# jrnerupudinho/Semi-Blind-Channel-Estimation-for-MIMO-RIS-communication-system-Using-EM-Algo

Hardware: NVIDIA B200
Metric: EM channel-estimation trials/sec (higher is better)
Workload: dtype f64

## Files before the change

semi-blind-channel-estimation-for-mimo-ris-communication-system-using-em-algo_b200/csrc/estep.cu:

```cuda
#include <math.h>

#include "common.cuh"
#include "tensor.cuh"

namespace sbce {

static __device__ __forceinline__ constexpr int cmax(int a, int b) { return a > b ? a : b; }

__global__ void k_pilot_stats(int n_tx, int total, const cplx* __restrict__ Xp, cplx* __restrict__ pm,
                              cplx* __restrict__ pR) {
    int s = blockIdx.x * blockDim.x + threadIdx.x;
    if (s >= total) return;
    const cplx* x = Xp + (size_t)s * n_tx;
    for (int i = 0; i < n_tx; ++i) {
        cplx xi = x[i];
        pm[(size_t)s * n_tx + i] = cconj(xi);
        for (int j = 0; j < n_tx; ++j) pR[((size_t)s * n_tx + i) * n_tx + j] = cmulc(x[j], xi);
    }
}

cudaError_t launch_pilot_stats(const Dims& d, int nb, const double* Xp, double* pil_m, double* pil_R, cudaStream_t s) {
    int total = nb * d.T_p;
    if (total == 0) return cudaSuccess;
    k_pilot_stats<<<(total + 127) / 128, 128, 0, s>>>(d.n_tx, total, (const cplx*)Xp, (cplx*)pil_m, (cplx*)pil_R);
    count_launch();
    return cudaGetLastError();
}

template <int NTX, int NRX>
__device__ __forceinline__ void heff_qr_finish(const Dims& d, int b, int t, cplx (&A)[cmax(NTX, NRX)][NTX],
                                               const cplx* __restrict__ Yd, const cplx* __restrict__ Xoff,
                                               double* __restrict__ qr) {
    constexpr int NR = cmax(NTX, NRX);
    cplx y[NR];
#pragma unroll
    for (int r = 0; r < NR; ++r) y[r] = (r < NRX) ? Yd[((size_t)b * d.T_d + t) * NRX + r] : mk(0.0, 0.0);
    if (Xoff != nullptr) {
        const cplx* o = Xoff + ((size_t)b * d.T_d + t) * NTX;
#pragma unroll
        for (int j = 0; j < NTX; ++j) {
            const cplx oj = o[j], noj = mk(-oj.x, -oj.y);
#pragma unroll
            for (int r = 0; r < NRX; ++r) cfma(y[r], A[r][j], noj);
        }
    }

#pragma unroll
    for (int k = 0; k < NTX; ++k) {
        double nrm2 = 0.0;
#pragma unroll
        for (int i = k; i < NR; ++i) nrm2 += cnorm2(A[i][k]);
        if (nrm2 > 0.0) {
            const double nrm = sqrt(nrm2);
            const cplx a0 = A[k][k];
            const double abs0 = sqrt(cnorm2(a0));
            const cplx phase = abs0 > 0.0 ? mk(a0.x / abs0, a0.y / abs0) : mk(1.0, 0.0);
            const cplx vk = cscale(phase, abs0 + nrm);
            const double beta = 1.0 / (nrm * (nrm + abs0));
#pragma unroll
            for (int c = k + 1; c <= NTX; ++c) {
                cplx w = mk(0.0, 0.0);
                if (c < NTX) {
                    cfmac(w, A[k][c], vk);
#pragma unroll
                    for (int i = k + 1; i < NR; ++i) cfmac(w, A[i][c], A[i][k]);
                    w = cscale(w, beta);
                    cplx nw = mk(-w.x, -w.y);
                    cfma(A[k][c], nw, vk);
#pragma unroll
                    for (int i = k + 1; i < NR; ++i) cfma(A[i][c], nw, A[i][k]);
                } else {
                    cfmac(w, y[k], vk);
#pragma unroll
                    for (int i = k + 1; i < NR; ++i) cfmac(w, y[i], A[i][k]);
                    w = cscale(w, beta);
                    cplx nw = mk(-w.x, -w.y);
                    cfma(y[k], nw, vk);
#pragma unroll
                    for (int i = k + 1; i < NR; ++i) cfma(y[i], nw, A[i][k]);
                }
            }
            const cplx rot = mk(-phase.x, phase.y);
#pragma unroll
            for (int c = k + 1; c < NTX; ++c) A[k][c] = cmul(A[k][c], rot);
            y[k] = cmul(y[k], rot);
            A[k][k] = mk(nrm, 0.0);
        } else {
            A[k][k] = mk(0.0, 0.0);
        }
    }

    double* rec = qr + ((size_t)b * d.T_d + t) * d.rec;
    int o = 0;
#pragma unroll
    for (int i = 0; i < NTX; ++i)
#pragma unroll
        for (int j = i; j < NTX; ++j) {
            rec[o++] = A[i][j].x;
            rec[o++] = (j == i) ? 0.0 : A[i][j].y;
        }
#pragma unroll
    for (int i = 0; i < NTX; ++i) {
        rec[o++] = y[i].x;
        rec[o++] = y[i].y;
    }
    double c0 = 0.0;
#pragma unroll
    for (int i = NTX; i < NR; ++i) c0 += cnorm2(y[i]);
    rec[o++] = c0;
    rec[o++] = 0.0;
}

template <int NTX, int NRX>
__global__ void __launch_bounds__(128) k_heff_qr(Dims d, const cplx* __restrict__ Yd, const cplx* __restrict__ PsiD,
                                                 const cplx* __restrict__ theta, const int32_t* __restrict__ active,
                                                 const cplx* __restrict__ Xoff, double* __restrict__ qr, int use_smem) {
    constexpr int NR = cmax(NTX, NRX);
    extern __shared__ double2 heff_smem[];
    const int b = blockIdx.y;
    if (active != nullptr && active[b] == 0) return;
    const cplx* th = theta + (size_t)b * d.L * NRX;
    if (use_smem) {
        for (int e = threadIdx.x; e < d.L * NRX; e += blockDim.x) heff_smem[e] = th[e];
        __syncthreads();
        th = heff_smem;
    }
    const int t = blockIdx.x * blockDim.x + threadIdx.x;
    if (t >= d.T_d) return;

    const cplx* psi = PsiD + ((size_t)(d.psi_shared ? 0 : b) * d.T_d + t) * d.N1;

    cplx A[NR][NTX];
#pragma unroll
    for (int r = 0; r < NR; ++r)
#pragma unroll
        for (int j = 0; j < NTX; ++j) A[r][j] = mk(0.0, 0.0);

#pragma unroll 4
    for (int n = 0; n < d.N1; ++n) {
        const cplx p = psi[n];
        const cplx* row = th + (size_t)n * NTX * NRX;
#pragma unroll
        for (int j = 0; j < NTX; ++j)
#pragma unroll
            for (int r = 0; r < NRX; ++r) cfma(A[r][j], p, row[j * NRX + r]);
    }
    heff_qr_finish<NTX, NRX>(d, b, t, A, Yd, Xoff, qr);
}

template <int NTX, int NRX>
__global__ void __launch_bounds__(128, 4) k_heff_qr_mma(Dims d, const cplx* __restrict__ Yd,
                                                        const cplx* __restrict__ PsiD, const cplx* __restrict__ theta,
                                                        const int32_t* __restrict__ active,
                                                        const cplx* __restrict__ Xoff, double* __restrict__ qr) {
    constexpr int NR = cmax(NTX, NRX);
    constexpr int NC = NTX * NRX;
    constexpr int NT = (NC + 7) / 8;
    constexpr int TS = NT * 8 + 2;
    constexpr int HS = NC + 1;
    extern __shared__ double2 heff_smem[];
    const int b = blockIdx.y;
    if (active != nullptr && active[b] == 0) return;
    const int N1 = d.N1, KP = (N1 + 7) & ~7;
    cplx* sTh = heff_smem;
    cplx* sH = sTh + KP * TS;
    {
        const cplx* th = theta + (size_t)b * d.L * NRX;
        for (int e = threadIdx.x; e < KP * TS; e += blockDim.x) {
            const int n = e / TS, c = e % TS;
            sTh[e] = (n < N1 && c < NC) ? th[n * NC + c] : mk(0.0, 0.0);
        }
    }
    __syncthreads();
    const int warp = threadIdx.x >> 5, lane = threadIdx.x & 31, g = lane >> 2, tig = lane & 3;
    const int t0 = blockIdx.x * 128 + warp * 32;
    if (t0 >= d.T_d) return;
    const cplx* psi_b = PsiD + (size_t)(d.psi_shared ? 0 : b) * d.T_d * N1;
    const cplx* prow[2][2];
#pragma unroll
    for (int mt = 0; mt < 2; ++mt)
#pragma unroll
        for (int h = 0; h < 2; ++h) prow[mt][h] = psi_b + (size_t)min(t0 + mt * 16 + g + 8 * h, d.T_d - 1) * N1;
    {
        const char* rowp = (const char*)(psi_b + (size_t)min(t0 + lane, d.T_d - 1) * N1);
        for (int o = 0; o < N1 * (int)sizeof(cplx); o += 128) asm volatile("prefetch.global.L2 [%0];" ::"l"(rowp + o));
    }
    double cr[2][NT][4], ci[2][NT][4];
#pragma unroll
    for (int mt = 0; mt < 2; ++mt)
#pragma unroll
        for (int nt = 0; nt < NT; ++nt)
#pragma unroll
            for (int e = 0; e < 4; ++e) { cr[mt][nt][e] = 0.0; ci[mt][nt][e] = 0.0; }
#pragma unroll 2
    for (int k0 = 0; k0 < KP; k0 += 8) {
        const int ka = k0 + tig, kb = ka + 4;
        const bool va = ka < N1, vb = kb < N1;
        double ar[2][4], ai[2][4];
#pragma unroll
        for (int mt = 0; mt < 2; ++mt) {
            const cplx a0 = va ? prow[mt][0][ka] : mk(0.0, 0.0), a1 = va ? prow[mt][1][ka] : mk(0.0, 0.0);
            const cplx a2 = vb ? prow[mt][0][kb] : mk(0.0, 0.0), a3 = vb ? prow[mt][1][kb] : mk(0.0, 0.0);
            ar[mt][0] = a0.x; ar[mt][1] = a1.x; ar[mt][2] = a2.x; ar[mt][3] = a3.x;
            ai[mt][0] = a0.y; ai[mt][1] = a1.y; ai[mt][2] = a2.y; ai[mt][3] = a3.y;
        }
#pragma unroll
        for (int nt = 0; nt < NT; ++nt) {
            const cplx b0 = sTh[ka * TS + 8 * nt + g], b1 = sTh[kb * TS + 8 * nt + g];
#pragma unroll
            for (int mt = 0; mt < 2; ++mt) {
                dmma16x8x8(cr[mt][nt], ar[mt], b0.x, b1.x);
                dmma16x8x8(ci[mt][nt], ar[mt], b0.y, b1.y);
                dmma16x8x8(cr[mt][nt], ai[mt], -b0.y, -b1.y);
                dmma16x8x8(ci[mt][nt], ai[mt], b0.x, b1.x);
            }
        }
    }
    cplx* H = sH + (size_t)warp * 32 * HS;
#pragma unroll
    for (int mt = 0; mt < 2; ++mt)
#pragma unroll
        for (int nt = 0; nt < NT; ++nt)
#pragma unroll
            for (int h = 0; h < 2; ++h) {
                const int row = mt * 16 + g + 8 * h, c = 8 * nt + 2 * tig;
                if (c < NC) H[row * HS + c] = mk(cr[mt][nt][2 * h], ci[mt][nt][2 * h]);
                if (c + 1 < NC) H[row * HS + c + 1] = mk(cr[mt][nt][2 * h + 1], ci[mt][nt][2 * h + 1]);
            }
    __syncwarp();
    const int t = t0 + lane;
    if (t >= d.T_d) return;
    cplx A[NR][NTX];
#pragma unroll
    for (int r = 0; r < NR; ++r)
#pragma unroll
        for (int j = 0; j < NTX; ++j) A[r][j] = (r < NRX) ? H[lane * HS + j * NRX + r] : mk(0.0, 0.0);
    heff_qr_finish<NTX, NRX>(d, b, t, A, Yd, Xoff, qr);
}

__device__ __forceinline__ double group8_sum(double v) {
    v += shfl_xor_d(v, 4);
    v += shfl_xor_d(v, 2);
    v += shfl_xor_d(v, 1);
    return v;
}

template <int NTX>
__global__ void __launch_bounds__(128) k_heff_qr_rows(Dims d, const cplx* __restrict__ Yd,
                                                      const cplx* __restrict__ PsiD, const cplx* __restrict__ theta,
                                                      const int32_t* __restrict__ active,
                                                      const cplx* __restrict__ Xoff, double* __restrict__ qr) {
    const int b = blockIdx.y;
    if (active != nullptr && active[b] == 0) return;
    const int r = threadIdx.x & 7;
    const int tq = blockIdx.x * (blockDim.x >> 3) + (threadIdx.x >> 3);
    const bool tv = tq < d.T_d;
    const int t = tv ? tq : d.T_d - 1;
    const int nrx = d.n_rx;
    const bool rv = r < nrx;
    const int rr = rv ? r : 0;

    const cplx* psi = PsiD + ((size_t)(d.psi_shared ? 0 : b) * d.T_d + t) * d.N1;
    const cplx* th = theta + (size_t)b * d.L * nrx;

    cplx A[NTX + 1];
#pragma unroll
    for (int j = 0; j <= NTX; ++j) A[j] = mk(0.0, 0.0);
#pragma unroll 2
    for (int n = 0; n < d.N1; ++n) {
        const cplx p = psi[n];
        const cplx* row = th + (size_t)n * NTX * nrx + rr;
#pragma unroll
        for (int j = 0; j < NTX; ++j) cfma(A[j], p, __ldg(&row[j * nrx]));
    }
    A[NTX] = Yd[((size_t)b * d.T_d + t) * nrx + rr];
    if (Xoff != nullptr) {
        const cplx* o = Xoff + ((size_t)b * d.T_d + t) * NTX;
#pragma unroll
        for (int j = 0; j < NTX; ++j) {
            const cplx oj = o[j];
            cfma(A[NTX], A[j], mk(-oj.x, -oj.y));
        }
    }
    if (!rv) {
#pragma unroll
        for (int j = 0; j <= NTX; ++j) A[j] = mk(0.0, 0.0);
    }

#pragma unroll
    for (int k = 0; k < NTX; ++k) {
        const double nrm2 = group8_sum(r >= k ? cnorm2(A[k]) : 0.0);
        const bool ok = nrm2 > 0.0;
        const double nrm = sqrt(nrm2);
        const int src = (threadIdx.x & 24) + k;
        const cplx a0 = mk(shfl_d(A[k].x, src), shfl_d(A[k].y, src));
        const double abs0 = sqrt(cnorm2(a0));
        const cplx phase = abs0 > 0.0 ? mk(a0.x / abs0, a0.y / abs0) : mk(1.0, 0.0);
        const cplx vk = cscale(phase, abs0 + nrm);
        const double beta = ok ? 1.0 / (nrm * (nrm + abs0)) : 0.0;
        const cplx vr = (r == k) ? vk : (r > k ? A[k] : mk(0.0, 0.0));
#pragma unroll
        for (int c = k + 1; c <= NTX; ++c) {
            cplx w = mk(0.0, 0.0);
            cfmac(w, A[c], vr);
            w = mk(group8_sum(w.x) * beta, group8_sum(w.y) * beta);
            const cplx nw = mk(-w.x, -w.y);
            cfma(A[c], nw, vr);
        }
        if (r == k) {
            const cplx rot = mk(-phase.x, phase.y);
#pragma unroll
            for (int c = k + 1; c <= NTX; ++c) A[c] = cmul(A[c], rot);
            A[k] = mk(ok ? nrm : 0.0, 0.0);
        }
    }
    const double c0 = group8_sum(r >= NTX ? cnorm2(A[NTX]) : 0.0);
    if (!tv) return;
    double* rec = qr + ((size_t)b * d.T_d + t) * d.rec;
    if (r < NTX) {
        double* o = rec + 2 * (r * NTX - (r * (r - 1)) / 2);
#pragma unroll
        for (int j = 0; j < NTX; ++j)
            if (j >= r) {
                o[2 * (j - r)] = A[j].x;
                o[2 * (j - r) + 1] = (j == r) ? 0.0 : A[j].y;
            }
        rec[NTX * (NTX + 1) + 2 * r] = A[NTX].x;
        rec[NTX * (NTX + 1) + 2 * r + 1] = A[NTX].y;
    }
    if (r == 0) {
        rec[NTX * (NTX + 1) + 2 * NTX] = c0;
        rec[NTX * (NTX + 1) + 2 * NTX + 1] = 0.0;
    }
}

constexpr double SBCE_THR = 64.0;
constexpr int ENUM_QCAP = 1024;

template <int NTX, int SQM>
struct EnumT {
    static constexpr int M = SQM * SQM;
    static constexpr int BITS = (SQM == 2 ? 2 : (SQM == 4 ? 4 : 6));
    static constexpr int HB = BITS / 2;
    static constexpr int NODE_STREAMS = NTX - 1;
    static constexpr int PLWANT = (5 + BITS - 1) / BITS;
    static constexpr int PL = NODE_STREAMS < PLWANT ? NODE_STREAMS : PLWANT;
    static constexpr int NPREF = 1 << (BITS * PL);
    static constexpr int NPAIR = NTX * (NTX - 1) / 2;
    static constexpr int NPAIR1 = NPAIR > 0 ? NPAIR : 1;
    static constexpr int NACC = 1 + 3 * NTX + 2 * NPAIR;
    static constexpr int O_TAB = 0;
    static constexpr int O_G = O_TAB + 2 * NPAIR1 * M;
    static constexpr int O_YT = O_G + NTX * SQM;
    static constexpr int O_C0 = O_YT + 2 * NTX;
    static constexpr int O_ACC = O_C0 + 1;
    static constexpr int O_AREF = O_ACC + NACC;
    static constexpr int O_S2 = O_AREF + 1;
    static constexpr int O_CNT = O_S2 + 1;
    static constexpr int O_Q = O_CNT + 1;
    static constexpr int O_SCR = O_Q + ENUM_QCAP / 2;
    static constexpr int WS_DOUBLES = ((O_SCR + NACC * 32) + 1) & ~1;

    __device__ __forceinline__ static double pam(int a) { return (double)(2 * a - SQM + 1); }
    __device__ __forceinline__ static cplx cval(int m) { return mk(pam(m & (SQM - 1)), pam(m >> HB)); }
    __device__ __forceinline__ static int pair(int i, int s) { return s * (s - 1) / 2 + i; }

    __device__ __forceinline__ static int slice(double v, const double* gs, double& dist) {
        int a = 0;
        double e = v - gs[0];
        dist = e * e;
#pragma unroll
        for (int q = 1; q < SQM; ++q) {
            e = v - gs[q];
            const double dq = e * e;
            if (dq < dist) { dist = dq; a = q; }
        }
        return a;
    }

    __device__ __forceinline__ static double fold(double v, double r) {
        double a = fabs(v);
        if (SQM == 8) a = fabs(a - 4.0 * r);
        if (SQM >= 4) a = fabs(a - 2.0 * r);
        return a - r;
    }
};

template <int NTX, int SQM>
__device__ __noinline__ void enum_flush(double* ws, double warp_best) {
    typedef EnumT<NTX, SQM> E;
    constexpr int M = E::M;
    const int lane = threadIdx.x & 31;
    __syncwarp();
    int* cntp = (int*)(ws + E::O_CNT);
    const int n = min(*cntp, ENUM_QCAP);
    const int* q = (const int*)(ws + E::O_Q);
    const cplx* tab = (const cplx*)(ws + E::O_TAB);
    const double* g = ws + E::O_G;
    const double inv_s2 = ws[E::O_S2];
    double aref = ws[E::O_AREF];
    if (warp_best < aref) {
        const double f = exp((warp_best - aref) * inv_s2);
        for (int i = lane; i < E::NACC; i += 32) ws[E::O_ACC + i] *= f;
        aref = warp_best;
    }
    double* A = ws + E::O_ACC;
    if (n <= 2) {
        constexpr int LG = (SQM == 2 ? 1 : (SQM == 4 ? 2 : 3));
        const int a = lane & (SQM - 1);
        const bool isQ = (lane >> LG) & 1;
        const double pq = E::pam(a);
        for (int e = 0; e < n; ++e) {
            const int code = q[e];
            double base = ws[E::O_C0];
            cplx t0;
            {
                cplx acc[NTX];
#pragma unroll
                for (int i = 0; i < NTX; ++i) acc[i] = mk(ws[E::O_YT + 2 * i], ws[E::O_YT + 2 * i + 1]);
#pragma unroll
                for (int s = NTX - 1; s >= 1; --s) {
                    const int m = (code >> (E::BITS * (NTX - 1 - s))) & (M - 1);
                    const double eI = acc[s].x - g[s * SQM + (m & (SQM - 1))];
                    const double eQ = acc[s].y - g[s * SQM + (m >> E::HB)];
                    base += fma(eI, eI, eQ * eQ);
#pragma unroll
                    for (int i = 0; i < NTX; ++i)
                        if (i < s) acc[i] = csub(acc[i], tab[E::pair(i, s) * M + m]);
                }
                t0 = acc[0];
            }
            const double ev = (isQ ? t0.y : t0.x) - g[a];
            const double dd = ev * ev;
            double mn = dd;
#pragma unroll
            for (int o = SQM / 2; o > 0; o >>= 1) mn = fmin(mn, shfl_xor_d(mn, o));
            const double w = exp((mn - dd) * inv_s2);
            double s0 = w, s1 = pq * w, s2 = pq * pq * w;
#pragma unroll
            for (int o = SQM / 2; o > 0; o >>= 1) {
                s0 += shfl_xor_d(s0, o);
                s1 += shfl_xor_d(s1, o);
                s2 += shfl_xor_d(s2, o);
            }
            const double o0 = shfl_xor_d(s0, SQM), o1 = shfl_xor_d(s1, SQM), o2 = shfl_xor_d(s2, SQM);
            const double om = shfl_xor_d(mn, SQM);
            const double EI = isQ ? o0 : s0, A1 = isQ ? o1 : s1, A2 = isQ ? o2 : s2, minI = isQ ? om : mn;
            const double EQ = isQ ? s0 : o0, B1 = isQ ? s1 : o1, B2 = isQ ? s2 : o2, minQ = isQ ? mn : om;
            const double W = exp((aref - (base + minI + minQ)) * inv_s2);
            const double E0 = W * EI * EQ;
            const cplx F0 = mk(W * A1 * EQ, -W * EI * B1);
            const double Q0 = W * (A2 * EQ + EI * B2);
            constexpr int NR = (E::NACC + 31) / 32;
            double mine[NR];
#pragma unroll
            for (int r = 0; r < NR; ++r) mine[r] = 0.0;
            auto add = [&](int idx, double v) { if ((idx & 31) == lane) mine[idx >> 5] = v; };
            add(0, E0);
            add(1, F0.x);
            add(1 + NTX, F0.y);
            add(1 + 2 * NTX, Q0);
#pragma unroll
            for (int s = 1; s < NTX; ++s) {
                const cplx xs = E::cval((code >> (E::BITS * (NTX - 1 - s))) & (M - 1));
                add(1 + s, E0 * xs.x);
                add(1 + NTX + s, -E0 * xs.y);
                add(1 + 2 * NTX + s, E0 * cnorm2(xs));
                const cplx v = cmul(F0, xs);
                add(1 + 3 * NTX + 2 * E::pair(0, s), v.x);
                add(1 + 3 * NTX + 2 * E::pair(0, s) + 1, v.y);
#pragma unroll
                for (int i = 1; i < NTX; ++i)
                    if (i < s) {
                        const cplx xi = E::cval((code >> (E::BITS * (NTX - 1 - i))) & (M - 1));
                        const cplx cx = cmulc(xs, xi);
                        add(1 + 3 * NTX + 2 * E::pair(i, s), E0 * cx.x);
                        add(1 + 3 * NTX + 2 * E::pair(i, s) + 1, E0 * cx.y);
                    }
            }
#pragma unroll
            for (int r = 0; r < NR; ++r)
                if (32 * r + lane < E::NACC) A[32 * r + lane] += mine[r];
            __syncwarp();
        }
        if (lane == 0) {
            ws[E::O_AREF] = aref;
            *cntp = 0;
        }
        __syncwarp();
        return;
    }
    double* scr = ws + E::O_SCR;
    int nround = 0;
    auto radd = [&](int idx, double v) { scr[idx * 32 + lane] = v; };
    for (int e0 = 0; e0 < n; e0 += 32) {
        const int e = e0 + lane;
        const bool have = e < n;
        nround = min(32, n - e0);
        const int code = have ? q[e] : 0;
        cplx t0;
        double base = ws[E::O_C0];
        {
            cplx acc[NTX];
#pragma unroll
            for (int i = 0; i < NTX; ++i) acc[i] = mk(ws[E::O_YT + 2 * i], ws[E::O_YT + 2 * i + 1]);
#pragma unroll
            for (int s = NTX - 1; s >= 1; --s) {
                const int m = (code >> (E::BITS * (NTX - 1 - s))) & (M - 1);
                const double eI = acc[s].x - g[s * SQM + (m & (SQM - 1))];
                const double eQ = acc[s].y - g[s * SQM + (m >> E::HB)];
                base += fma(eI, eI, eQ * eQ);
#pragma unroll
                for (int i = 0; i < NTX; ++i)
                    if (i < s) acc[i] = csub(acc[i], tab[E::pair(i, s) * M + m]);
            }
            t0 = acc[0];
        }
        double minI = 1e300, minQ = 1e300;
#pragma unroll
        for (int a = 0; a < SQM; ++a) {
            const double eI = t0.x - g[a], eQ = t0.y - g[a];
            minI = fmin(minI, eI * eI);
            minQ = fmin(minQ, eQ * eQ);
        }
        const double W = have ? exp((aref - (base + minI + minQ)) * inv_s2) : 0.0;
        double EI = 0, A1 = 0, A2 = 0, EQ = 0, B1 = 0, B2 = 0;
#pragma unroll 1
        for (int a = 0; a < SQM; ++a) {
            const double pq = E::pam(a);
            const double eI = t0.x - g[a], eQ = t0.y - g[a];
            const double wI = exp((minI - eI * eI) * inv_s2), wQ = exp((minQ - eQ * eQ) * inv_s2);
            EI += wI; A1 = fma(pq, wI, A1); A2 = fma(pq * pq, wI, A2);
            EQ += wQ; B1 = fma(pq, wQ, B1); B2 = fma(pq * pq, wQ, B2);
        }
        const double E0 = W * EI * EQ;
        const cplx F0 = mk(W * A1 * EQ, -W * EI * B1);
        const double Q0 = W * (A2 * EQ + EI * B2);
        radd(0, E0);
        radd(1, F0.x);
        radd(1 + NTX, F0.y);
        radd(1 + 2 * NTX, Q0);
#pragma unroll
        for (int s = 1; s < NTX; ++s) {
            const cplx xs = E::cval((code >> (E::BITS * (NTX - 1 - s))) & (M - 1));
            radd(1 + s, E0 * xs.x);
            radd(1 + NTX + s, -E0 * xs.y);
            radd(1 + 2 * NTX + s, E0 * cnorm2(xs));
            const cplx v = cmul(F0, xs);
            radd(1 + 3 * NTX + 2 * E::pair(0, s), v.x);
            radd(1 + 3 * NTX + 2 * E::pair(0, s) + 1, v.y);
#pragma unroll
            for (int i = 1; i < NTX; ++i)
                if (i < s) {
                    const cplx xi = E::cval((code >> (E::BITS * (NTX - 1 - i))) & (M - 1));
                    const cplx cx = cmulc(xs, xi);
                    radd(1 + 3 * NTX + 2 * E::pair(i, s), E0 * cx.x);
                    radd(1 + 3 * NTX + 2 * E::pair(i, s) + 1, E0 * cx.y);
                }
        }
        __syncwarp();
        for (int i = lane; i < E::NACC; i += 32) {
            double acc = 0.0;
            for (int e2 = 0; e2 < nround; ++e2) acc += scr[i * 32 + e2];
            A[i] += acc;
        }
        __syncwarp();
    }
    __syncwarp();
    if (lane == 0) {
        ws[E::O_AREF] = aref;
        *cntp = 0;
    }
    __syncwarp();
}

template <int NTX, int SQM, bool HARD>
struct Scan {
    typedef EnumT<NTX, SQM> E;
    static constexpr int M = E::M;
    double* ws;
    const cplx* tab;
    const double* g;
    double r0;
    double thr;
    double best, lim;
    int bestk;
    bool prune;

    __device__ __forceinline__ void leaf(cplx t0, double nb, int code) {
        const double fI = E::fold(t0.x, r0), fQ = E::fold(t0.y, r0);
        const double nodemin = fma(fI, fI, fma(fQ, fQ, nb));
        if (nodemin <= lim) {
            if (nodemin <= best) {
                double dI, dQ;
                const int iI = E::slice(t0.x, g, dI), iQ = E::slice(t0.y, g, dQ);
                const double val = nb + dI + dQ;
                const int k = code + ((iQ * SQM + iI) << (E::BITS * (NTX - 1)));
                if (val < best || (val == best && k < bestk)) {
                    best = val;
                    bestk = k;
                    lim = HARD ? val : val + thr;
                }
            }
            if (!HARD) {
                int* cntp = (int*)(ws + E::O_CNT);
                const int slot = atomicAdd(cntp, 1);
                if (slot < ENUM_QCAP) ((int*)(ws + E::O_Q))[slot] = code;
            }
        }
    }

    __device__ __forceinline__ void maybe_flush() {
        if (!HARD) {
            __syncwarp();
            const int c = *(volatile int*)(ws + E::O_CNT);
            if (c > ENUM_QCAP - 32 * SQM) {
                double wb = best;
#pragma unroll
                for (int o = 16; o > 0; o >>= 1) wb = fmin(wb, shfl_xor_d(wb, o));
                enum_flush<NTX, SQM>(ws, wb);
            }
        }
    }


    template <int S_>
    __device__ __forceinline__ void inner(const cplx (&acc)[NTX], double base, int code, cplx r01, bool dead) {
        dead = dead || (prune && base > lim);
        if constexpr (S_ == 0) {
            if (!dead) leaf(acc[0], base, code);
        } else if constexpr (S_ == 1) {
            if (__all_sync(0xffffffffu, dead)) return;
            const double* g1 = g + SQM;
            double dI1[SQM];
#pragma unroll
            for (int a = 0; a < SQM; ++a) {
                const double eI = acc[1].x - g1[a];
                dI1[a] = eI * eI;
            }
#pragma unroll 1
            for (int iQ = 0; iQ < SQM; ++iQ) {
                const double eQ = acc[1].y - g1[iQ];
                const double bq = base + __dmul_rn(eQ, eQ);
                const bool deadq = dead || (prune && bq > lim);
                if (__all_sync(0xffffffffu, deadq)) continue;
                const double pQ = E::pam(iQ);
                const cplx tq = mk(fma(pQ, r01.y, acc[0].x), fma(-pQ, r01.x, acc[0].y));
                const int cq = code + ((iQ * SQM) << (E::BITS * (NTX - 2)));
                if (!deadq) {
#pragma unroll
                    for (int iI = 0; iI < SQM; ++iI) {
                        const double pI = E::pam(iI);
                        const cplx t0 = mk(fma(-pI, r01.x, tq.x), fma(-pI, r01.y, tq.y));
                        leaf(t0, bq + dI1[iI], cq + (iI << (E::BITS * (NTX - 2))));
                    }
                }
                maybe_flush();
            }
        } else {
            if (__all_sync(0xffffffffu, dead)) return;
#pragma unroll 1
            for (int m = 0; m < M; ++m) {
                const double* gs = g + S_ * SQM;
                const double eI = acc[S_].x - gs[m & (SQM - 1)];
                const double eQ = acc[S_].y - gs[m >> E::HB];
                const double nb = base + fma(eI, eI, eQ * eQ);
                cplx nacc[NTX];
#pragma unroll
                for (int i = 0; i < NTX; ++i) nacc[i] = (i < S_) ? csub(acc[i], tab[E::pair(i, S_) * M + m]) : acc[i];
                inner<S_ - 1>(nacc, nb, code + (m << (E::BITS * (NTX - 1 - S_))), r01, dead);
            }
        }
    }

    template <int S_, int LEFT>
    __device__ __forceinline__ void prefix(const cplx (&acc)[NTX], double base, int code, int p, cplx r01, bool dead) {
        if constexpr (LEFT == 0) {
            inner<S_>(acc, base, code, r01, dead);
        } else {
            const int m = (p >> (E::BITS * (LEFT - 1))) & (M - 1);
            const double* gs = g + S_ * SQM;
            const double eI = acc[S_].x - gs[m & (SQM - 1)];
            const double eQ = acc[S_].y - gs[m >> E::HB];
            const double nb = base + fma(eI, eI, eQ * eQ);
            cplx nacc[NTX];
#pragma unroll
            for (int i = 0; i < NTX; ++i) nacc[i] = (i < S_) ? csub(acc[i], tab[E::pair(i, S_) * M + m]) : acc[i];
            prefix<S_ - 1, LEFT - 1>(nacc, nb, code + (m << (E::BITS * (NTX - 1 - S_))), p, r01, dead);
        }
    }
};

template <int NTX, int SQM, bool HARD, int WARPS>
__global__ void __launch_bounds__(WARPS * 32, (NTX > 4 ? 2 : 4)) k_enum(Dims d, const double* __restrict__ qr,
                                                     const double* __restrict__ varn,
                                                     const int32_t* __restrict__ active, cplx* __restrict__ stat_m,
                                                     cplx* __restrict__ stat_R, int32_t* __restrict__ kstar,
                                                     double* __restrict__ lse_sym) {
    typedef EnumT<NTX, SQM> E;
    constexpr int M = E::M;
    extern __shared__ __align__(16) double enum_smem[];
    const int b = blockIdx.y;
    const int warp = threadIdx.x >> 5, lane = threadIdx.x & 31;
    const int t = blockIdx.x * WARPS + warp;
    if (t >= d.T_d) return;
    const double* grec = qr + ((size_t)b * d.T_d + t) * d.rec;
    const int32_t act = (active != nullptr) ? active[b] : 1;
    const double vn = varn[b];
    const double rec0 = (lane < d.rec) ? grec[lane] : 0.0;
    if (act == 0) return;

    double* ws = enum_smem + (size_t)warp * E::WS_DOUBLES;
    cplx* tab = (cplx*)(ws + E::O_TAB);
    double* g = ws + E::O_G;
    const double* rec = ws + E::O_SCR;
    {
        if (lane < d.rec) ws[E::O_SCR + lane] = rec0;
        for (int i = lane + 32; i < d.rec; i += 32) ws[E::O_SCR + i] = grec[i];
        __syncwarp();
    }
    cplx yt[NTX];
    cplx r01 = mk(0.0, 0.0);
    double r00;
    {
        cplx Rm[NTX][NTX];
        int o = 0;
#pragma unroll
        for (int i = 0; i < NTX; ++i)
#pragma unroll
            for (int j = i; j < NTX; ++j) {
                Rm[i][j] = mk(rec[o], rec[o + 1]);
                o += 2;
            }
#pragma unroll
        for (int i = 0; i < NTX; ++i) {
            yt[i] = mk(rec[o], rec[o + 1]);
            o += 2;
        }
        r00 = Rm[0][0].x;
        if (NTX > 1) r01 = Rm[0][NTX > 1 ? 1 : 0];
#pragma unroll
        for (int s = 1; s < NTX; ++s)
#pragma unroll
            for (int i = 0; i < s; ++i)
                for (int m = lane; m < M; m += 32) tab[E::pair(i, s) * M + m] = cmul(Rm[i][s], E::cval(m));
        if (lane < NTX * SQM) {
            const int s = lane / SQM, a = lane % SQM;
            double dd = 0.0;
#pragma unroll
            for (int q = 0; q < NTX; ++q)
                if (q == s) dd = Rm[q][q].x;
            g[lane] = dd * E::pam(a);
        }
    }
    const double c0 = rec[NTX * (NTX + 1) + 2 * NTX];
    const double s2 = vn * vn, inv_s2 = 1.0 / s2;
    if (lane == 0) {
#pragma unroll
        for (int i = 0; i < NTX; ++i) {
            ws[E::O_YT + 2 * i] = yt[i].x;
            ws[E::O_YT + 2 * i + 1] = yt[i].y;
        }
        ws[E::O_C0] = c0;
        ws[E::O_AREF] = 1e300;
        ws[E::O_S2] = inv_s2;
        *(int*)(ws + E::O_CNT) = 0;
    }
    for (int i = lane; i < E::NACC; i += 32) ws[E::O_ACC + i] = 0.0;
    __syncwarp();

    Scan<NTX, SQM, HARD> sc;
    sc.ws = ws;
    sc.tab = tab;
    sc.g = g;
    sc.r0 = r00;
    sc.thr = SBCE_THR * s2;
    sc.prune = (d.flags & SBCE_FLAG_FULL_SCAN) == 0;
    {
        cplx acc[NTX];
#pragma unroll
        for (int i = 0; i < NTX; ++i) acc[i] = yt[i];
        double base = c0;
        int k = 0;
#pragma unroll
        for (int s = NTX - 1; s >= 0; --s) {
            double dI, dQ;
            const int iI = E::slice(acc[s].x, g + s * SQM, dI), iQ = E::slice(acc[s].y, g + s * SQM, dQ);
            const int m = iQ * SQM + iI;
            base += dI + dQ;
            k += m << (E::BITS * (NTX - 1 - s));
#pragma unroll
            for (int i = 0; i < NTX; ++i)
                if (i < s) acc[i] = csub(acc[i], tab[E::pair(i, s) * M + m]);
        }
        sc.best = base;
        sc.bestk = k;
        sc.lim = HARD ? base : base + sc.thr;
    }

    unsigned top_alive = 0xffffffffu;
    constexpr int TOP_SHIFT = E::BITS * (E::PL - 1);
    if (E::PL >= 2 && sc.prune) {
        bool a = false;
        if (lane < M) {
            const double* gs = g + (NTX - 1) * SQM;
            const double eI = yt[NTX - 1].x - gs[lane & (SQM - 1)];
            const double eQ = yt[NTX - 1].y - gs[lane >> E::HB];
            a = !(c0 + fma(eI, eI, eQ * eQ) > sc.lim);
        }
        top_alive = __ballot_sync(0xffffffffu, a);
    }
    for (int pb = 0; pb < E::NPREF; pb += 32) {
        if (E::PL >= 2) {
            const int lo = pb >> TOP_SHIFT, hi = min(pb + 31, E::NPREF - 1) >> TOP_SHIFT;
            const unsigned bits = (hi >= 31 ? 0xffffffffu : ((2u << hi) - 1u)) & ~((1u << lo) - 1u);
            if ((top_alive & bits) == 0u) continue;
        }
        const int p = pb + lane;
        const bool valid = p < E::NPREF;
        sc.template prefix<NTX - 1, E::PL>(yt, c0, 0, valid ? p : 0, r01, !valid);
    }

    double best = sc.best;
    int bestk = sc.bestk;
#pragma unroll
    for (int o = 16; o > 0; o >>= 1) {
        const double ob = shfl_xor_d(best, o);
        const int ok = __shfl_xor_sync(0xffffffffu, bestk, o);
        if (ob < best || (ob == best && ok < bestk)) { best = ob; bestk = ok; }
    }
    const size_t sidx = (size_t)b * d.T_d + t;
    if (kstar != nullptr && lane == 0) kstar[sidx] = bestk;

    bool collapsed = HARD;
    double S = 0.0;
    if (!HARD) {
        enum_flush<NTX, SQM>(ws, best);
        S = ws[E::O_ACC];
        if (!(S > 0.0) || !isfinite(S)) collapsed = true;
    }
    if (collapsed) {
        if (lane == 0) {
            cplx xs[NTX];
#pragma unroll
            for (int s = 0; s < NTX; ++s) xs[s] = E::cval((bestk >> (E::BITS * (NTX - 1 - s))) & (M - 1));
#pragma unroll
            for (int i = 0; i < NTX; ++i) {
                stat_m[sidx * NTX + i] = cconj(xs[i]);
#pragma unroll
                for (int j = 0; j < NTX; ++j) stat_R[(sidx * NTX + i) * NTX + j] = cmulc(xs[j], xs[i]);
            }
            if (lse_sym != nullptr) lse_sym[sidx] = -best * inv_s2;
        }
        return;
    }
    {
        const double invS = 1.0 / S;
        const double* A = ws + E::O_ACC;
        for (int l = lane; l < NTX * NTX; l += 32) {
            const int i = l / NTX, j = l % NTX;
            cplx v;
            if (i == j) {
                v = mk(A[1 + 2 * NTX + j] * invS, 0.0);
            } else {
                const int lo = min(i, j), hi = max(i, j);
                const int pr = 1 + 3 * NTX + 2 * E::pair(lo, hi);
                const double a = A[pr] * invS, c = A[pr + 1] * invS;
                v = mk(a, i < j ? c : -c);
            }
            stat_R[sidx * NTX * NTX + l] = v;
        }
        if (lane < NTX) stat_m[sidx * NTX + lane] = mk(A[1 + lane] * invS, A[1 + NTX + lane] * invS);
        if (lse_sym != nullptr && lane == 0) lse_sym[sidx] = -ws[E::O_AREF] * inv_s2 + log(S);
    }
}

__global__ void k_superimpose_stats(Dims d, int nb, const cplx* __restrict__ Xoff, const int32_t* __restrict__ active,
                                    cplx* __restrict__ stat_m, cplx* __restrict__ stat_R) {
    const int s = blockIdx.x * blockDim.x + threadIdx.x;
    if (s >= nb * d.T_d) return;
    if (active != nullptr && active[s / d.T_d] == 0) return;
    const int n = d.n_tx;
    const cplx* o = Xoff + (size_t)s * n;
    cplx* m = stat_m + (size_t)s * n;
    cplx* R = stat_R + (size_t)s * n * n;
    for (int i = 0; i < n; ++i)
        for (int j = 0; j < n; ++j) {
            cplx v = R[i * n + j];
            cfma(v, m[i], o[j]);
            v = cadd(v, cconj(cmul(o[i], m[j])));
            v = cadd(v, cmulc(o[j], o[i]));
            R[i * n + j] = v;
        }
    for (int i = 0; i < n; ++i) m[i] = cadd(m[i], cconj(o[i]));
}

cudaError_t launch_superimpose_stats(const Dims& d, int nb, const double* Xoff, const int32_t* active, double* stat_m,
                                     double* stat_R, cudaStream_t s) {
    const int total = nb * d.T_d;
    k_superimpose_stats<<<(total + 127) / 128, 128, 0, s>>>(d, nb, (const cplx*)Xoff, active, (cplx*)stat_m, (cplx*)stat_R);
    count_launch();
    return cudaGetLastError();
}

template <int NTX, int NRX>
static cudaError_t run_heff(const Dims& d, int nb, const double* Yd, const double* PsiD, const double* theta,
                            const int32_t* active, const double* Xoff, double* qr, cudaStream_t s) {
    static SmemOptIn optin_mma, optin;
    dim3 grid((d.T_d + 127) / 128, nb);
    constexpr int NC = NTX * NRX, NT = (NC + 7) / 8;
    const int KP = (d.N1 + 7) & ~7;
    const size_t smem_mma = sizeof(cplx) * ((size_t)KP * (NT * 8 + 2) + 4 * 32 * (NC + 1));
    if (NC >= 8 && d.N1 >= 16 && smem_mma <= 100 * 1024) {
        cudaError_t e = opt_in_smem(optin_mma, (const void*)k_heff_qr_mma<NTX, NRX>, smem_mma);
        if (e != cudaSuccess) return e;
        k_heff_qr_mma<NTX, NRX><<<grid, 128, smem_mma, s>>>(d, (const cplx*)Yd, (const cplx*)PsiD, (const cplx*)theta,
                                                            active, (const cplx*)Xoff, qr);
        count_launch();
        return cudaGetLastError();
    }
    size_t smem = sizeof(cplx) * (size_t)d.L * NRX;
    const int use_smem = smem <= 64 * 1024;
    if (!use_smem) smem = 0;
    cudaError_t e = opt_in_smem(optin, (const void*)k_heff_qr<NTX, NRX>, smem);
    if (e != cudaSuccess) return e;
    k_heff_qr<NTX, NRX><<<grid, 128, smem, s>>>(d, (const cplx*)Yd, (const cplx*)PsiD, (const cplx*)theta, active,
                                                (const cplx*)Xoff, qr, use_smem);
    count_launch();
    return cudaGetLastError();
}

template <int NTX>
static cudaError_t run_heff_ntx(const Dims& d, int nb, const double* Yd, const double* PsiD, const double* theta,
                                const int32_t* active, const double* Xoff, double* qr, cudaStream_t s) {
    switch (d.n_rx) {
        case 1: return run_heff<NTX, 1>(d, nb, Yd, PsiD, theta, active, Xoff, qr, s);
        case 2: return run_heff<NTX, 2>(d, nb, Yd, PsiD, theta, active, Xoff, qr, s);
        case 3: return run_heff<NTX, 3>(d, nb, Yd, PsiD, theta, active, Xoff, qr, s);
        case 4: return run_heff<NTX, 4>(d, nb, Yd, PsiD, theta, active, Xoff, qr, s);
        case 6: return run_heff<NTX, 6>(d, nb, Yd, PsiD, theta, active, Xoff, qr, s);
        case 8: return run_heff<NTX, 8>(d, nb, Yd, PsiD, theta, active, Xoff, qr, s);
        default: return cudaErrorInvalidValue;
    }
}

template <int NTX, int SQM>
static cudaError_t run_enum(const Dims& d, int nb, const double* qr, const double* varn, const int32_t* active,
                            double* stat_m, double* stat_R, int32_t* kstar, double* lse_sym, cudaStream_t s) {
    constexpr int WARPS = 4;
    dim3 grid((d.T_d + WARPS - 1) / WARPS, nb);
    constexpr size_t smem = sizeof(double) * WARPS * EnumT<NTX, SQM>::WS_DOUBLES;
    static SmemOptIn optin_hard, optin_soft;
    cudaError_t e;
    if (d.mode == SBCE_MODE_HARD) {
        e = opt_in_smem(optin_hard, (const void*)k_enum<NTX, SQM, true, WARPS>, smem);
        if (e != cudaSuccess) return e;
        k_enum<NTX, SQM, true, WARPS><<<grid, WARPS * 32, smem, s>>>(d, qr, varn, active, (cplx*)stat_m,
                                                                      (cplx*)stat_R, kstar, lse_sym);
    } else {
        e = opt_in_smem(optin_soft, (const void*)k_enum<NTX, SQM, false, WARPS>, smem);
        if (e != cudaSuccess) return e;
        k_enum<NTX, SQM, false, WARPS><<<grid, WARPS * 32, smem, s>>>(d, qr, varn, active, (cplx*)stat_m,
                                                                       (cplx*)stat_R, kstar, lse_sym);
    }
    count_launch();
    return cudaGetLastError();
}

template <int NTX>
static cudaError_t run_heff_rows(const Dims& d, int nb, const double* Yd, const double* PsiD, const double* theta,
                                 const int32_t* active, const double* Xoff, double* qr, cudaStream_t s) {
    dim3 grid((d.T_d + 15) / 16, nb);
    k_heff_qr_rows<NTX><<<grid, 128, 0, s>>>(d, (const cplx*)Yd, (const cplx*)PsiD, (const cplx*)theta, active,
                                             (const cplx*)Xoff, qr);
    count_launch();
    return cudaGetLastError();
}

template <int NTX>
static cudaError_t run_enum_wide(const Dims& d, int nb, const double* qr, const double* varn, const int32_t* active,
                                 double* stat_m, double* stat_R, int32_t* kstar, double* lse_sym, cudaStream_t s) {
    if (d.sqM == 2) return run_enum<NTX, 2>(d, nb, qr, varn, active, stat_m, stat_R, kstar, lse_sym, s);
    if constexpr (NTX <= 6) {
        if (d.sqM == 4) return run_enum<NTX, 4>(d, nb, qr, varn, active, stat_m, stat_R, kstar, lse_sym, s);
    }
    return cudaErrorInvalidValue;
}

template <int NTX>
static cudaError_t run_enum_ntx(const Dims& d, int nb, const double* qr, const double* varn, const int32_t* active,
                                double* stat_m, double* stat_R, int32_t* kstar, double* lse_sym, cudaStream_t s) {
    switch (d.sqM) {
        case 2: return run_enum<NTX, 2>(d, nb, qr, varn, active, stat_m, stat_R, kstar, lse_sym, s);
        case 4: return run_enum<NTX, 4>(d, nb, qr, varn, active, stat_m, stat_R, kstar, lse_sym, s);
        case 8: return run_enum<NTX, 8>(d, nb, qr, varn, active, stat_m, stat_R, kstar, lse_sym, s);
        default: return cudaErrorInvalidValue;
    }
}

cudaError_t launch_heff_qr(const Dims& d, int nb, const double* Yd, const double* PsiD, const double* theta,
                           const int32_t* active, const double* Xoff, double* qr, cudaStream_t s) {
    switch (d.n_tx) {
        case 1: return run_heff_ntx<1>(d, nb, Yd, PsiD, theta, active, Xoff, qr, s);
        case 2: return run_heff_ntx<2>(d, nb, Yd, PsiD, theta, active, Xoff, qr, s);
        case 3: return run_heff_ntx<3>(d, nb, Yd, PsiD, theta, active, Xoff, qr, s);
        case 4: return run_heff_ntx<4>(d, nb, Yd, PsiD, theta, active, Xoff, qr, s);
        case 5: return run_heff_rows<5>(d, nb, Yd, PsiD, theta, active, Xoff, qr, s);
        case 6: return run_heff_rows<6>(d, nb, Yd, PsiD, theta, active, Xoff, qr, s);
        case 7: return run_heff_rows<7>(d, nb, Yd, PsiD, theta, active, Xoff, qr, s);
        case 8: return run_heff_rows<8>(d, nb, Yd, PsiD, theta, active, Xoff, qr, s);
        default: return cudaErrorInvalidValue;
    }
}

cudaError_t launch_enum(const Dims& d, int nb, const double* qr, const double* varn, const int32_t* active,
                        double* stat_m, double* stat_R, int32_t* kstar, double* lse_sym, cudaStream_t s) {
    switch (d.n_tx) {
        case 1: return run_enum_ntx<1>(d, nb, qr, varn, active, stat_m, stat_R, kstar, lse_sym, s);
        case 2: return run_enum_ntx<2>(d, nb, qr, varn, active, stat_m, stat_R, kstar, lse_sym, s);
        case 3: return run_enum_ntx<3>(d, nb, qr, varn, active, stat_m, stat_R, kstar, lse_sym, s);
        case 4: return run_enum_ntx<4>(d, nb, qr, varn, active, stat_m, stat_R, kstar, lse_sym, s);
        case 5: return run_enum_wide<5>(d, nb, qr, varn, active, stat_m, stat_R, kstar, lse_sym, s);
        case 6: return run_enum_wide<6>(d, nb, qr, varn, active, stat_m, stat_R, kstar, lse_sym, s);
        case 7: return run_enum_wide<7>(d, nb, qr, varn, active, stat_m, stat_R, kstar, lse_sym, s);
        case 8: return run_enum_wide<8>(d, nb, qr, varn, active, stat_m, stat_R, kstar, lse_sym, s);
        default: return cudaErrorInvalidValue;
    }
}

}
```

Before: 23350.

## Split warps into half-warp groups for small-NTX sphere enumeration

For NTX<=4 each received symbol is now enumerated by a 16-lane half-warp instead of a full warp, so each warp handles two symbols with per-group masks, shuffles, and workspaces. Queue capacity and flush thresholds scale with the group size. Prefix rounds are now skipped through a bitmask of live rounds. Node-level flushing is batched when the queue can hold a whole node. This aims to reduce idle lanes when the prefix tree is small, at the cost of more shared memory per block and more serial work per lane.

```diff
diff --git a/semi-blind-channel-estimation-for-mimo-ris-communication-system-using-em-algo_b200/csrc/estep.cu b/semi-blind-channel-estimation-for-mimo-ris-communication-system-using-em-algo_b200/csrc/estep.cu
--- a/semi-blind-channel-estimation-for-mimo-ris-communication-system-using-em-algo_b200/csrc/estep.cu
+++ b/semi-blind-channel-estimation-for-mimo-ris-communication-system-using-em-algo_b200/csrc/estep.cu
@@ -335,7 +335,7 @@
 }
 
 constexpr double SBCE_THR = 64.0;
-constexpr int ENUM_QCAP = 1024;
+__device__ __forceinline__ double shfl_xor_h(unsigned hm, double v, int o) { return __shfl_xor_sync(hm, v, o); }
 
 template <int NTX, int SQM>
 struct EnumT {
@@ -349,6 +349,12 @@
     static constexpr int NPAIR = NTX * (NTX - 1) / 2;
     static constexpr int NPAIR1 = NPAIR > 0 ? NPAIR : 1;
     static constexpr int NACC = 1 + 3 * NTX + 2 * NPAIR;
+    static constexpr int REC = NTX * (NTX + 1) + 2 * NTX + 2;
+    static constexpr int G = NTX > 4 ? 32 : 16;
+    static constexpr int QCAP = G == 32 ? 1024 : 480;
+    __device__ __forceinline__ static unsigned gmask() { return G == 32 ? 0xffffffffu : 0xFFFFu << (threadIdx.x & 16); }
+    __device__ __forceinline__ static int glane() { return threadIdx.x & (G - 1); }
+    __device__ __forceinline__ static int gshift() { return threadIdx.x & (32 - G); }
     static constexpr int O_TAB = 0;
     static constexpr int O_G = O_TAB + 2 * NPAIR1 * M;
     static constexpr int O_YT = O_G + NTX * SQM;
@@ -358,8 +364,12 @@
     static constexpr int O_S2 = O_AREF + 1;
     static constexpr int O_CNT = O_S2 + 1;
     static constexpr int O_Q = O_CNT + 1;
-    static constexpr int O_SCR = O_Q + ENUM_QCAP / 2;
-    static constexpr int WS_DOUBLES = ((O_SCR + NACC * 32) + 1) & ~1;
+    static constexpr int O_SCR = O_Q + QCAP / 2;
+    static constexpr int WS_DOUBLES = ((O_SCR + NACC * G) + 1) & ~1;
+    static_assert(NACC * G >= REC, "the QR record is staged in the flush scratch");
+    static_assert(PL < NODE_STREAMS || NPREF <= QCAP, "prefix-only trees must fit the queue without a flush");
+    static_assert(G * SQM < QCAP, "maybe_flush threshold");
+    static_assert(PL < 2 || M <= G, "pre-pass: one lane per top symbol");
 
     __device__ __forceinline__ static double pam(int a) { return (double)(2 * a - SQM + 1); }
     __device__ __forceinline__ static cplx cval(int m) { return mk(pam(m & (SQM - 1)), pam(m >> HB)); }
@@ -390,10 +400,11 @@
 __device__ __noinline__ void enum_flush(double* ws, double warp_best) {
     typedef EnumT<NTX, SQM> E;
     constexpr int M = E::M;
-    const int lane = threadIdx.x & 31;
-    __syncwarp();
+    const int lane = E::glane();
+    const unsigned hm = E::gmask();
+    __syncwarp(hm);
     int* cntp = (int*)(ws + E::O_CNT);
-    const int n = min(*cntp, ENUM_QCAP);
+    const int n = min(*cntp, E::QCAP);
     const int* q = (const int*)(ws + E::O_Q);
     const cplx* tab = (const cplx*)(ws + E::O_TAB);
     const double* g = ws + E::O_G;
@@ -401,7 +412,7 @@
     double aref = ws[E::O_AREF];
     if (warp_best < aref) {
         const double f = exp((warp_best - aref) * inv_s2);
-        for (int i = lane; i < E::NACC; i += 32) ws[E::O_ACC + i] *= f;
+        for (int i = lane; i < E::NACC; i += E::G) ws[E::O_ACC + i] *= f;
         aref = warp_best;
     }
     double* A = ws + E::O_ACC;
@@ -434,28 +445,28 @@
             const double dd = ev * ev;
             double mn = dd;
 #pragma unroll
-            for (int o = SQM / 2; o > 0; o >>= 1) mn = fmin(mn, shfl_xor_d(mn, o));
+            for (int o = SQM / 2; o > 0; o >>= 1) mn = fmin(mn, shfl_xor_h(hm, mn, o));
             const double w = exp((mn - dd) * inv_s2);
             double s0 = w, s1 = pq * w, s2 = pq * pq * w;
 #pragma unroll
             for (int o = SQM / 2; o > 0; o >>= 1) {
-                s0 += shfl_xor_d(s0, o);
-                s1 += shfl_xor_d(s1, o);
-                s2 += shfl_xor_d(s2, o);
-            }
-            const double o0 = shfl_xor_d(s0, SQM), o1 = shfl_xor_d(s1, SQM), o2 = shfl_xor_d(s2, SQM);
-            const double om = shfl_xor_d(mn, SQM);
+                s0 += shfl_xor_h(hm, s0, o);
+                s1 += shfl_xor_h(hm, s1, o);
+                s2 += shfl_xor_h(hm, s2, o);
+            }
+            const double o0 = shfl_xor_h(hm, s0, SQM), o1 = shfl_xor_h(hm, s1, SQM), o2 = shfl_xor_h(hm, s2, SQM);
+            const double om = shfl_xor_h(hm, mn, SQM);
             const double EI = isQ ? o0 : s0, A1 = isQ ? o1 : s1, A2 = isQ ? o2 : s2, minI = isQ ? om : mn;
             const double EQ = isQ ? s0 : o0, B1 = isQ ? s1 : o1, B2 = isQ ? s2 : o2, minQ = isQ ? mn : om;
             const double W = exp((aref - (base + minI + minQ)) * inv_s2);
             const double E0 = W * EI * EQ;
             const cplx F0 = mk(W * A1 * EQ, -W * EI * B1);
             const double Q0 = W * (A2 * EQ + EI * B2);
-            constexpr int NR = (E::NACC + 31) / 32;
+            constexpr int NR = (E::NACC + E::G - 1) / E::G;
             double mine[NR];
 #pragma unroll
             for (int r = 0; r < NR; ++r) mine[r] = 0.0;
-            auto add = [&](int idx, double v) { if ((idx & 31) == lane) mine[idx >> 5] = v; };
+            auto add = [&](int idx, double v) { if ((idx & (E::G - 1)) == lane) mine[idx / E::G] = v; };
             add(0, E0);
             add(1, F0.x);
             add(1 + NTX, F0.y);
@@ -480,23 +491,23 @@
             }
 #pragma unroll
             for (int r = 0; r < NR; ++r)
-                if (32 * r + lane < E::NACC) A[32 * r + lane] += mine[r];
-            __syncwarp();
+                if (E::G * r + lane < E::NACC) A[E::G * r + lane] += mine[r];
+            __syncwarp(hm);
         }
         if (lane == 0) {
             ws[E::O_AREF] = aref;
             *cntp = 0;
         }
-        __syncwarp();
+        __syncwarp(hm);
         return;
     }
     double* scr = ws + E::O_SCR;
     int nround = 0;
-    auto radd = [&](int idx, double v) { scr[idx * 32 + lane] = v; };
-    for (int e0 = 0; e0 < n; e0 += 32) {
+    auto radd = [&](int idx, double v) { scr[idx * E::G + lane] = v; };
+    for (int e0 = 0; e0 < n; e0 += E::G) {
         const int e = e0 + lane;
         const bool have = e < n;
-        nround = min(32, n - e0);
+        nround = min(E::G, n - e0);
         const int code = have ? q[e] : 0;
         cplx t0;
         double base = ws[E::O_C0];
@@ -558,20 +569,20 @@
                     radd(1 + 3 * NTX + 2 * E::pair(i, s) + 1, E0 * cx.y);
                 }
         }
-        __syncwarp();
-        for (int i = lane; i < E::NACC; i += 32) {
+        __syncwarp(hm);
+        for (int i = lane; i < E::NACC; i += E::G) {
             double acc = 0.0;
-            for (int e2 = 0; e2 < nround; ++e2) acc += scr[i * 32 + e2];
+            for (int e2 = 0; e2 < nround; ++e2) acc += scr[i * E::G + e2];
             A[i] += acc;
         }
-        __syncwarp();
-    }
-    __syncwarp();
+        __syncwarp(hm);
+    }
+    __syncwarp(hm);
     if (lane == 0) {
         ws[E::O_AREF] = aref;
         *cntp = 0;
     }
-    __syncwarp();
+    __syncwarp(hm);
 }
 
 template <int NTX, int SQM, bool HARD>
@@ -605,19 +616,21 @@
             if (!HARD) {
                 int* cntp = (int*)(ws + E::O_CNT);
                 const int slot = atomicAdd(cntp, 1);
-                if (slot < ENUM_QCAP) ((int*)(ws + E::O_Q))[slot] = code;
-            }
-        }
-    }
-
+                if (slot < E::QCAP) ((int*)(ws + E::O_Q))[slot] = code;
+            }
+        }
+    }
+
+    template <int PER_LANE>
     __device__ __forceinline__ void maybe_flush() {
         if (!HARD) {
-            __syncwarp();
+            const unsigned hm = E::gmask();
+            __syncwarp(hm);
             const int c = *(volatile int*)(ws + E::O_CNT);
-            if (c > ENUM_QCAP - 32 * SQM) {
+            if (c > E::QCAP - E::G * PER_LANE) {
                 double wb = best;
 #pragma unroll
-                for (int o = 16; o > 0; o >>= 1) wb = fmin(wb, shfl_xor_d(wb, o));
+                for (int o = E::G / 2; o > 0; o >>= 1) wb = fmin(wb, shfl_xor_h(hm, wb, o));
                 enum_flush<NTX, SQM>(ws, wb);
             }
         }
@@ -630,7 +643,8 @@
         if constexpr (S_ == 0) {
             if (!dead) leaf(acc[0], base, code);
         } else if constexpr (S_ == 1) {
-            if (__all_sync(0xffffffffu, dead)) return;
+            if (__all_sync(E::gmask(), dead)) return;
+            constexpr bool NODE_FLUSH = E::G * M < E::QCAP;
             const double* g1 = g + SQM;
             double dI1[SQM];
 #pragma unroll
@@ -643,7 +657,7 @@
                 const double eQ = acc[1].y - g1[iQ];
                 const double bq = base + __dmul_rn(eQ, eQ);
                 const bool deadq = dead || (prune && bq > lim);
-                if (__all_sync(0xffffffffu, deadq)) continue;
+                if (__all_sync(E::gmask(), deadq)) continue;
                 const double pQ = E::pam(iQ);
                 const cplx tq = mk(fma(pQ, r01.y, acc[0].x), fma(-pQ, r01.x, acc[0].y));
                 const int cq = code + ((iQ * SQM) << (E::BITS * (NTX - 2)));
@@ -655,10 +669,11 @@
                         leaf(t0, bq + dI1[iI], cq + (iI << (E::BITS * (NTX - 2))));
                     }
                 }
-                maybe_flush();
-            }
+                if (!NODE_FLUSH) maybe_flush<SQM>();
+            }
+            if (NODE_FLUSH) maybe_flush<M>();
         } else {
-            if (__all_sync(0xffffffffu, dead)) return;
+            if (__all_sync(E::gmask(), dead)) return;
 #pragma unroll 1
             for (int m = 0; m < M; ++m) {
                 const double* gs = g + S_ * SQM;
@@ -701,23 +716,24 @@
     constexpr int M = E::M;
     extern __shared__ __align__(16) double enum_smem[];
     const int b = blockIdx.y;
-    const int warp = threadIdx.x >> 5, lane = threadIdx.x & 31;
-    const int t = blockIdx.x * WARPS + warp;
+    constexpr int SPW = 32 / E::G;
+    const int warp = threadIdx.x >> 5, sub = (threadIdx.x & 31) / E::G, gl = E::glane();
+    const int t = (blockIdx.x * WARPS + warp) * SPW + sub;
     if (t >= d.T_d) return;
     const double* grec = qr + ((size_t)b * d.T_d + t) * d.rec;
     const int32_t act = (active != nullptr) ? active[b] : 1;
     const double vn = varn[b];
-    const double rec0 = (lane < d.rec) ? grec[lane] : 0.0;
+    const double rec0 = (gl < E::REC) ? grec[gl] : 0.0;
     if (act == 0) return;
 
-    double* ws = enum_smem + (size_t)warp * E::WS_DOUBLES;
+    double* ws = enum_smem + (size_t)(SPW * warp + sub) * E::WS_DOUBLES;
     cplx* tab = (cplx*)(ws + E::O_TAB);
     double* g = ws + E::O_G;
     const double* rec = ws + E::O_SCR;
     {
-        if (lane < d.rec) ws[E::O_SCR + lane] = rec0;
-        for (int i = lane + 32; i < d.rec; i += 32) ws[E::O_SCR + i] = grec[i];
-        __syncwarp();
+        if (gl < E::REC) ws[E::O_SCR + gl] = rec0;
+        for (int i = gl + E::G; i < E::REC; i += E::G) ws[E::O_SCR + i] = grec[i];
+        __syncwarp(E::gmask());
     }
     cplx yt[NTX];
     cplx r01 = mk(0.0, 0.0);
@@ -743,19 +759,15 @@
         for (int s = 1; s < NTX; ++s)
 #pragma unroll
             for (int i = 0; i < s; ++i)
-                for (int m = lane; m < M; m += 32) tab[E::pair(i, s) * M + m] = cmul(Rm[i][s], E::cval(m));
-        if (lane < NTX * SQM) {
-            const int s = lane / SQM, a = lane % SQM;
-            double dd = 0.0;
-#pragma unroll
-            for (int q = 0; q < NTX; ++q)
-                if (q == s) dd = Rm[q][q].x;
-            g[lane] = dd * E::pam(a);
+                for (int m = gl; m < M; m += E::G) tab[E::pair(i, s) * M + m] = cmul(Rm[i][s], E::cval(m));
+        if (gl < SQM) {
+#pragma unroll
+            for (int s = 0; s < NTX; ++s) g[s * SQM + gl] = Rm[s][s].x * E::pam(gl);
         }
     }
     const double c0 = rec[NTX * (NTX + 1) + 2 * NTX];
     const double s2 = vn * vn, inv_s2 = 1.0 / s2;
-    if (lane == 0) {
+    if (gl == 0) {
 #pragma unroll
         for (int i = 0; i < NTX; ++i) {
             ws[E::O_YT + 2 * i] = yt[i].x;
@@ -766,8 +778,8 @@
         ws[E::O_S2] = inv_s2;
         *(int*)(ws + E::O_CNT) = 0;
     }
-    for (int i = lane; i < E::NACC; i += 32) ws[E::O_ACC + i] = 0.0;
-    __syncwarp();
+    for (int i = gl; i < E::NACC; i += E::G) ws[E::O_ACC + i] = 0.0;
+    __syncwarp(E::gmask());
 
     Scan<NTX, SQM, HARD> sc;
     sc.ws = ws;
@@ -798,39 +810,46 @@
         sc.lim = HARD ? base : base + sc.thr;
     }
 
-    unsigned top_alive = 0xffffffffu;
-    constexpr int TOP_SHIFT = E::BITS * (E::PL - 1);
+    constexpr int NROUND = (E::NPREF + E::G - 1) / E::G;
+    static_assert(NROUND <= 32, "one bit per round");
+    unsigned live = NROUND == 32 ? 0xffffffffu : (1u << NROUND) - 1u;
     if (E::PL >= 2 && sc.prune) {
+        constexpr int TOP_SHIFT = E::BITS * (E::PL - 1);
         bool a = false;
-        if (lane < M) {
+        if (gl < M) {
             const double* gs = g + (NTX - 1) * SQM;
-            const double eI = yt[NTX - 1].x - gs[lane & (SQM - 1)];
-            const double eQ = yt[NTX - 1].y - gs[lane >> E::HB];
+            const double eI = yt[NTX - 1].x - gs[gl & (SQM - 1)];
+            const double eQ = yt[NTX - 1].y - gs[gl >> E::HB];
             a = !(c0 + fma(eI, eI, eQ * eQ) > sc.lim);
         }
-        top_alive = __ballot_sync(0xffffffffu, a);
-    }
-    for (int pb = 0; pb < E::NPREF; pb += 32) {
-        if (E::PL >= 2) {
-            const int lo = pb >> TOP_SHIFT, hi = min(pb + 31, E::NPREF - 1) >> TOP_SHIFT;
-            const unsigned bits = (hi >= 31 ? 0xffffffffu : ((2u << hi) - 1u)) & ~((1u << lo) - 1u);
-            if ((top_alive & bits) == 0u) continue;
-        }
-        const int p = pb + lane;
+        const unsigned top_alive = __ballot_sync(E::gmask(), a) >> E::gshift();
+        live = 0u;
+#pragma unroll
+        for (int r = 0; r < NROUND; ++r) {
+            const int lo = (E::G * r) >> TOP_SHIFT, hi = min(E::G * r + E::G - 1, E::NPREF - 1) >> TOP_SHIFT;
+            const unsigned bits = ((2u << hi) - 1u) & ~((1u << lo) - 1u);
+            if (top_alive & bits) live |= 1u << r;
+        }
+    }
+    while (live != 0u) {
+        const int pb = E::G * (__ffs(live) - 1);
+        live &= live - 1u;
+        const int p = pb + gl;
         const bool valid = p < E::NPREF;
         sc.template prefix<NTX - 1, E::PL>(yt, c0, 0, valid ? p : 0, r01, !valid);
     }
 
     double best = sc.best;
     int bestk = sc.bestk;
-#pragma unroll
-    for (int o = 16; o > 0; o >>= 1) {
-        const double ob = shfl_xor_d(best, o);
-        const int ok = __shfl_xor_sync(0xffffffffu, bestk, o);
+    const unsigned hm = E::gmask();
+#pragma unroll
+    for (int o = E::G / 2; o > 0; o >>= 1) {
+        const double ob = shfl_xor_h(hm, best, o);
+        const int ok = __shfl_xor_sync(hm, bestk, o);
         if (ob < best || (ob == best && ok < bestk)) { best = ob; bestk = ok; }
     }
     const size_t sidx = (size_t)b * d.T_d + t;
-    if (kstar != nullptr && lane == 0) kstar[sidx] = bestk;
+    if (kstar != nullptr && gl == 0) kstar[sidx] = bestk;
 
     bool collapsed = HARD;
     double S = 0.0;
@@ -840,7 +859,7 @@
         if (!(S > 0.0) || !isfinite(S)) collapsed = true;
     }
     if (collapsed) {
-        if (lane == 0) {
+        if (gl == 0) {
             cplx xs[NTX];
 #pragma unroll
             for (int s = 0; s < NTX; ++s) xs[s] = E::cval((bestk >> (E::BITS * (NTX - 1 - s))) & (M - 1));
@@ -857,7 +876,7 @@
     {
         const double invS = 1.0 / S;
         const double* A = ws + E::O_ACC;
-        for (int l = lane; l < NTX * NTX; l += 32) {
+        for (int l = gl; l < NTX * NTX; l += E::G) {
             const int i = l / NTX, j = l % NTX;
             cplx v;
             if (i == j) {
@@ -870,8 +889,8 @@
             }
             stat_R[sidx * NTX * NTX + l] = v;
         }
-        if (lane < NTX) stat_m[sidx * NTX + lane] = mk(A[1 + lane] * invS, A[1 + NTX + lane] * invS);
-        if (lse_sym != nullptr && lane == 0) lse_sym[sidx] = -ws[E::O_AREF] * inv_s2 + log(S);
+        if (gl < NTX) stat_m[sidx * NTX + gl] = mk(A[1 + gl] * invS, A[1 + NTX + gl] * invS);
+        if (lse_sym != nullptr && gl == 0) lse_sym[sidx] = -ws[E::O_AREF] * inv_s2 + log(S);
     }
 }
 
@@ -947,9 +966,10 @@
 template <int NTX, int SQM>
 static cudaError_t run_enum(const Dims& d, int nb, const double* qr, const double* varn, const int32_t* active,
                             double* stat_m, double* stat_R, int32_t* kstar, double* lse_sym, cudaStream_t s) {
-    constexpr int WARPS = 4;
-    dim3 grid((d.T_d + WARPS - 1) / WARPS, nb);
-    constexpr size_t smem = sizeof(double) * WARPS * EnumT<NTX, SQM>::WS_DOUBLES;
+    typedef EnumT<NTX, SQM> E;
+    constexpr int WARPS = 4, SYMS = WARPS * 32 / E::G;
+    dim3 grid((d.T_d + SYMS - 1) / SYMS, nb);
+    constexpr size_t smem = sizeof(double) * SYMS * E::WS_DOUBLES;
     static SmemOptIn optin_hard, optin_soft;
     cudaError_t e;
     if (d.mode == SBCE_MODE_HARD) {
```

After: 24380 (median of 6 runs). +4.4%, better.
